# alexrich021/3dvnet

Measured on AMD Instinct MI355X. Metric: depth maps/sec (256x320, 96 planes, 7 src), higher is better.
Workload: dtype f32 storage/accumulate; MFMA operands split-bf16x3 (hi*hi+hi*lo+lo*hi, 16 mantissa bits); warp/variance f32 VALU; 1 GPU; cfg2: ScanNet-shape 256x320, 1 ref + 7 src (8 edges/ref), 96 planes, 56x56 plane grid, 32-ch quarter features 64x80; fused warp+variance -> CostRegNet -> soft-argmin depth (rows A1-A6); n_img_per_gpu=71, edges_per_ref=8, parallelism=single GPU, launch=eager, ranks_seen=1

## Files before the change

3dvnet_amd/build.py:

```python
import glob
import hashlib
import os
import subprocess
import sys

HERE = os.path.dirname(os.path.abspath(__file__))
ROOT = os.path.dirname(HERE)
CSRC = os.path.join(HERE, 'csrc')
LIB = os.path.join(HERE, 'lib3dvnet_hip.so')
HIPCC = os.environ.get('HIPCC', '/opt/rocm/bin/hipcc')
FLAGS = ['--offload-arch=gfx950', '-O3', '-std=c++17', '-fPIC', '-Wall', '-Wno-unused-function',
         '-I', os.path.join(ROOT, 'include'), '-I', CSRC] + os.environ.get('V3D_EXTRA_FLAGS', '').split()


def sources():
    return sorted(glob.glob(os.path.join(CSRC, '*.hip')))


def _flags_tag():
    return hashlib.sha256(' '.join([HIPCC] + FLAGS).encode()).hexdigest()[:12]


def _stale(target, deps):
    if not os.path.exists(target):
        return True
    t = os.path.getmtime(target)
    return any(os.path.getmtime(d) > t for d in deps)


def build(force=False, verbose=False, strict=False):
    headers = glob.glob(os.path.join(CSRC, '*.h')) + glob.glob(os.path.join(ROOT, 'include', '*.h'))
    tag = _flags_tag()
    objdir = os.path.join(HERE, 'build', tag)
    os.makedirs(objdir, exist_ok=True)
    stamp = os.path.join(HERE, 'build', 'linked_flags')
    linked = open(stamp).read().strip() if os.path.exists(stamp) else None
    procs, objs = [], []
    for src in sources():
        obj = os.path.join(objdir, os.path.basename(src)[:-4] + '.o')
        objs.append(obj)
        if force or _stale(obj, [src] + headers):
            cmd = [HIPCC] + FLAGS + ['-c', src, '-o', obj]
            if verbose:
                print(' '.join(cmd))
            procs.append((src, subprocess.Popen(cmd, stdout=subprocess.PIPE, stderr=subprocess.STDOUT)))
    for src, p in procs:
        out, _ = p.communicate()
        if p.returncode != 0:
            sys.stderr.write(out.decode())
            raise RuntimeError('hipcc failed on %s' % src)
        if verbose and out:
            print(out.decode())
    if not os.environ.get('V3D_EXTRA_FLAGS', '').strip() and not os.environ.get('V3D_SKIP_LDS_CHECK'):
        sys.path.insert(0, HERE)
        try:
            import isa_check
            isa_check.check(os.path.join(objdir, 'decoder.o'), strict=strict)
            isa_check.check_wide_lds(os.path.join(objdir, 'irb.o'), 'irb_kernel', strict=strict)
            isa_check.check_wide_lds(os.path.join(objdir, 'fpn.o'), 'fpn_level_kernel', strict=strict)
            isa_check.check_wide_lds(os.path.join(objdir, 'propz.o'), 'propz_kernel', strict=strict)
            isa_check.check_no_scratch(os.path.join(objdir, 'fusion.o'), 'fuse_depths_kernel', strict=strict)
            isa_check.check_no_scratch(os.path.join(objdir, 'tsdf.o'), 'tsdf_integrate_kernel', strict=strict)
            isa_check.check_no_scratch(os.path.join(objdir, 'tsdf_resample.o'), 'tsdf_resample_kernel', strict=strict)
            isa_check.check_no_scratch(os.path.join(objdir, 'tsdf_resample.o'), 'volume_resample_nearest_kernel', strict=strict)
            isa_check.check_no_scratch(os.path.join(objdir, 'cloudmetrics.o'), 'nn_query_kernel', strict=strict)
            isa_check.check_no_scratch(os.path.join(objdir, 'mesh.o'), 'mc_[a-z_]*_kernel', strict=strict)
            isa_check.check_no_scratch(os.path.join(objdir, 'meshrender.o'), 'mesh_render_kernel', strict=strict)
            isa_check.check_no_scratch(os.path.join(objdir, 'psv_variance.o'), 'psv_variance_window_kernel', strict=strict)
            isa_check.check_no_scratch(os.path.join(objdir, 'confidence.o'), 'soft_argmin_prob_kernel', strict=strict)
            isa_check.check_no_scratch(os.path.join(objdir, 'confidence.o'), 'prob_gather_kernel', strict=strict)
        finally:
            sys.path.pop(0)
    if force or procs or linked != tag or _stale(LIB, objs):
        cmd = [HIPCC, '--offload-arch=gfx950', '-shared', '-fPIC', '-o', LIB] + objs
        if verbose:
            print(' '.join(cmd))
        subprocess.check_call(cmd)
        with open(stamp, 'w') as f:
            f.write(tag + '\n')
    return LIB


if __name__ == '__main__':
    print(build(force='--force' in sys.argv, verbose='--verbose' in sys.argv))
```

3dvnet_amd/csrc/api.hip:

```cpp
#include <atomic>
#include <cstring>
#include <map>
#include <mutex>
#include <string>
#include <vector>

#include "v3d_common.h"

extern "C" int v3d_version(void) { return 9; }

extern "C" const char* v3d_last_error(void) { return v3d::err_buf(); }

namespace {
struct Span { std::string name; hipEvent_t a, b; };
std::mutex g_mu;
bool g_on = false;
std::vector<Span> g_spans;
std::vector<hipEvent_t> g_pool;
hipEvent_t take_event() {
  if (!g_pool.empty()) { hipEvent_t e = g_pool.back(); g_pool.pop_back(); return e; }
  hipEvent_t e; (void)hipEventCreate(&e); return e;
}
}

namespace v3d {
bool timing_enabled() { return g_on; }
void timing_begin(const char* name, hipStream_t s) {
  std::lock_guard<std::mutex> lk(g_mu);
  Span sp{name, take_event(), take_event()};
  (void)hipEventRecord(sp.a, s);
  g_spans.push_back(sp);
}
void timing_end(hipStream_t s) {
  std::lock_guard<std::mutex> lk(g_mu);
  if (!g_spans.empty()) (void)hipEventRecord(g_spans.back().b, s);
}
}

namespace {
struct OptDef { const char* name; int def; };
const OptDef kOptDefs[v3d::kOptCount] = {{"psv_kernel", 0}, {"c12_march", 1}, {"stop_after", 99}, {"gemm_rounds", 1},
                                         {"gemm_pipe", 1}, {"psv_walk", 0}, {"render_coop", 64}};
std::atomic<int> g_opt[v3d::kOptCount];
std::atomic<bool> g_opt_init{false};
void opt_init() {
  if (!g_opt_init.load(std::memory_order_acquire)) {
    std::lock_guard<std::mutex> lk(g_mu);
    if (!g_opt_init.load()) {
      for (int i = 0; i < v3d::kOptCount; ++i) g_opt[i].store(kOptDefs[i].def);
      g_opt_init.store(true, std::memory_order_release);
    }
  }
}
}

int v3d::option(v3d::Option o) {
  opt_init();
  return g_opt[o].load(std::memory_order_relaxed);
}

extern "C" int v3d_set_option(const char* name, int value) {
  V3D_REQUIRE(name, V3D_ERR_BAD_ARG, "v3d_set_option: null name");
  opt_init();
  for (int i = 0; i < v3d::kOptCount; ++i)
    if (!strcmp(name, kOptDefs[i].name)) {
      V3D_REQUIRE(!(i == v3d::kOptGemmRounds || i == v3d::kOptGemmPipe) || value == 0 || value == 1, V3D_ERR_BAD_ARG,
                  "v3d_set_option: %s must be 0 or 1 (got %d)", name, value);
      V3D_REQUIRE(!(i == v3d::kOptPsvWalk || i == v3d::kOptRenderCoop) || value >= 0, V3D_ERR_BAD_ARG,
                  "v3d_set_option: %s must be >= 0 (got %d)", name, value);
      g_opt[i].store(value);
      return V3D_OK;
    }
  return v3d::fail(V3D_ERR_BAD_ARG, "v3d_set_option: unknown option '%s'", name);
}

extern "C" int v3d_get_option(const char* name, int* value) {
  V3D_REQUIRE(name && value, V3D_ERR_BAD_ARG, "v3d_get_option: null argument");
  opt_init();
  for (int i = 0; i < v3d::kOptCount; ++i)
    if (!strcmp(name, kOptDefs[i].name)) { *value = g_opt[i].load(); return V3D_OK; }
  return v3d::fail(V3D_ERR_BAD_ARG, "v3d_get_option: unknown option '%s'", name);
}

extern "C" int v3d_timing_enable(int on) {
  std::lock_guard<std::mutex> lk(g_mu);
  g_on = on != 0;
  return V3D_OK;
}

extern "C" int v3d_timing_collect(int max_entries, char* names, int name_stride, float* total_ms,
                                  int* launches) {
  std::lock_guard<std::mutex> lk(g_mu);
  std::map<std::string, std::pair<float, int>> agg;
  std::vector<std::string> order;
  for (auto& sp : g_spans) {
    float ms = 0.f;
    if (hipEventSynchronize(sp.b) == hipSuccess) (void)hipEventElapsedTime(&ms, sp.a, sp.b);
    if (!agg.count(sp.name)) order.push_back(sp.name);
    agg[sp.name].first += ms;
    agg[sp.name].second += 1;
    g_pool.push_back(sp.a);
    g_pool.push_back(sp.b);
  }
  g_spans.clear();
  int n = 0;
  for (auto& k : order) {
    if (n >= max_entries) break;
    if (names && name_stride > 0) {
      strncpy(names + (size_t)n * name_stride, k.c_str(), name_stride - 1);
      names[(size_t)n * name_stride + name_stride - 1] = 0;
    }
    if (total_ms) total_ms[n] = agg[k].first;
    if (launches) launches[n] = agg[k].second;
    ++n;
  }
  return n;
}
```

3dvnet_amd/csrc/costreg.hip:

```cpp
#include <cstdlib>
#include <type_traits>
#include <vector>

#include "v3d_common.h"
#include "weight_pack.h"

#ifndef V3D_ABLATE
#define V3D_ABLATE 0
#endif

namespace {

typedef float f32x4 __attribute__((ext_vector_type(4)));
typedef float f32x2 __attribute__((ext_vector_type(2)));

enum { kConvS1 = 0, kConvS2 = 1, kDeconvS2 = 2, kConvS1Pair = 3 };

#ifdef V3D_PHASE_TIMING
constexpr int kPhaseSlots = 1 << 16;
__device__ unsigned long long g_phase[8 * kPhaseSlots];
#define PHASE_DECL                                  \
  long long ph_t = __builtin_readcyclecounter();    \
  long long ph_acc[8] = {0, 0, 0, 0, 0, 0, 0, 0}
#define PHASE_MARK(i)                                   \
// ... 754 lines not shown
        }
      }
      __syncthreads();
      const size_t out_plane = (size_t)p.Do * p.Ho * p.Wo;
      constexpr int QPR = C0::TW / 4, NQ = 8 * C0::TD * C0::TH * QPR;
#pragma unroll
      for (int k = 0; k < (NQ + NT - 1) / NT; ++k) {
        const int i = k * NT + tid;
        if (i >= NQ) break;
        const int co = i / (C0::TD * C0::TH * QPR), rem = i % (C0::TD * C0::TH * QPR);
        const int row = rem / QPR, q = rem % QPR;
        const int gz = oz0 + row / C0::TH, gy = oy0 + row % C0::TH, gx = ox0 + 4 * q;
        if (gz >= p.Do || gy >= p.Ho || gx >= p.Wo) continue;
        f32x4 v = *reinterpret_cast<const f32x4*>(os + co * OCS + row * C0::TW + 4 * q);
        const size_t o = ((size_t)n * 8 + co) * out_plane + ((size_t)gz * p.Ho + gy) * p.Wo + gx;
        if (gx + 3 < p.Wo && (p.Wo & 3) == 0) {
          if (p.skip) { const f32x4 sk = *reinterpret_cast<const f32x4*>(p.skip + o); v += sk; }
          *reinterpret_cast<f32x4*>(p.out + o) = v;
        } else {
          for (int e = 0; e < 4 && gx + e < p.Wo; ++e) p.out[o + e] = v[e] + (p.skip ? p.skip[o + e] : 0.f);
        }
      }
      PHASE_MARK(6);
    }
    cur = nxt;
  }
  PHASE_FLUSH;
}

enum { kOutF32 = 1, kOutSplit = 2 };

template <int CIN_, int COUT_, int STRIDE_, int WB_, int OUT_>
struct CG {
  static constexpr int CIN = CIN_, COUT = COUT_, S = STRIDE_, WB = WB_, OUT = OUT_;
  static constexpr int NCH = CIN / 8, NCG = COUT / 16;
  static constexpr int NRB = 16 / WB;
#ifndef V3D_CG_TD_S1
#define V3D_CG_TD_S1 4
#endif
#ifndef V3D_CG_TD_S2
#define V3D_CG_TD_S2 3
#endif
  static constexpr int TD = WB != 14 ? (S == 2 ? 2 : 4) : S == 2 ? V3D_CG_TD_S2 : V3D_CG_TD_S1, TH = 4 * NRB, TW = WB;
  static constexpr int NKZ = 3;
  static constexpr int ID = S * (TD - 1) + 3, IH = S * (TH - 1) + 3, IW = S * (TW - 1) + 3;
  static constexpr int NVOX = ID * IH * IW, NVOXP = NVOX + 8;
  static constexpr int WQ = NKZ * 3 * 2 * 64;
  static constexpr int NVO = TD * TH * TW;
  static constexpr int LPR = IW <= 16 ? 16 : 32, RPI = 256 / LPR;
  static constexpr int NROWS = 2 * ID * IH, NIT = (NROWS + RPI - 1) / RPI;
  static constexpr int NWIT = (WQ + 255) / 256;
  static constexpr size_t LDS_BYTES = (size_t)(2 * NVOXP + WQ) * 16;
  static constexpr bool PERSIST = NCH == 1;
  static constexpr int OCC = 2;
  static_assert(CIN % 8 == 0 && COUT % 16 == 0 && (WB == 14 || WB == 8), "shape");
  static_assert((size_t)NVO * 64 <= LDS_BYTES, "split output staging fits in the workgroup's LDS");
  static_assert((size_t)16 * (NVO + 2) * 4 <= LDS_BYTES, "fp32 output staging fits in the workgroup's LDS");
  static_assert((NROWS + RPI) * ID * IH < (1 << 20) && 4 * NVO * NVO < (1 << 20), "v3d::small_div ranges of the staging / output index");
};

struct ConvGParams {
  const void* in;
  const void* wp;
  const float* bias;
  float* out_f32;
  void* out_split;
  int n, Di, Hi, Wi, Do, Ho, Wo, ntz, nty, ntx;
  unsigned m_tx, m_ty, m_tz;
};

template <class C>
__global__ __launch_bounds__(256, C::OCC) void convg_bf16x2_kernel(ConvGParams p, const float* __restrict__ bias_r) {
  extern __shared__ __attribute__((aligned(16))) unsigned char smem[];
  u32x4* const xs = reinterpret_cast<u32x4*>(smem);
  u32x4* const wq = xs + 2 * C::NVOXP;
  const int tid = threadIdx.x, lane = tid & 63;
  const int wave = __builtin_amdgcn_readfirstlane(tid >> 6);
  const int kq = lane >> 4, jn = lane & 15;
  const size_t in_plane = (size_t)p.Di * p.Hi * p.Wi;
  const size_t out_plane = (size_t)p.Do * p.Ho * p.Wo;

  struct Item { int cg, n, oz0, oy0, ox0; };
  auto decode = [&](int t) __attribute__((always_inline)) {
    Item q;
    const unsigned t0 = (unsigned)t / C::NCG;
    q.cg = (int)((unsigned)t - t0 * C::NCG);
    const unsigned t1 = v3d::udiv_magic(t0, (unsigned)p.ntx, p.m_tx), t2 = v3d::udiv_magic(t1, (unsigned)p.nty, p.m_ty);
    const unsigned t3 = v3d::udiv_magic(t2, (unsigned)p.ntz, p.m_tz);
    q.ox0 = (int)(t0 - t1 * (unsigned)p.ntx) * C::TW;
    q.oy0 = (int)(t1 - t2 * (unsigned)p.nty) * C::TH;
    q.oz0 = (int)(t2 - t3 * (unsigned)p.ntz) * C::TD;
    q.n = (int)t3;
    return q;
  };
  const v3d::TileWalk walk = v3d::xcd_tile_walk(p.n * p.ntz * p.nty * p.ntx * C::NCG);
  if (walk.t >= walk.end) return;

  const int lrow = tid / C::LPR, lx = tid % C::LPR;
  const bool xok = lx < C::IW;
  u32x4 pre[C::NIT], wreg[C::NWIT];
  constexpr bool XPRE = C::PERSIST;
  auto issue = [&](const Item& q, int chunk) __attribute__((always_inline)) {
    const int iz0 = C::S * q.oz0 - 1, iy0 = C::S * q.oy0 - 1, sgx = C::S * q.ox0 - 1 + lx;
    const bool xin = xok && sgx >= 0 && sgx < p.Wi;
    const int sxc = min(max(sgx, 0), p.Wi - 1);
    const char* const ins = reinterpret_cast<const char*>(reinterpret_cast<const u32x4*>(p.in) +
                                                          ((size_t)q.n * C::NCH + chunk) * 2 * in_plane);
    const u32x4* const wg = reinterpret_cast<const u32x4*>(p.wp) + (size_t)q.cg * C::NCH * C::WQ;
#pragma unroll
    for (int it = 0; it < C::NIT; ++it) {
      const unsigned rr = (unsigned)(it * C::RPI + lrow);
      const unsigned part = v3d::small_div<C::ID * C::IH>(rr), rem = rr - part * (C::ID * C::IH);
      const unsigned rz = v3d::small_div<C::IH>(rem), ry = rem - rz * C::IH;
      const int gz = iz0 + (int)rz, gy = iy0 + (int)ry;
      const bool ok = rr < C::NROWS && xin && gz >= 0 && gz < p.Di && gy >= 0 && gy < p.Hi;
      const int zc = min(max(gz, 0), p.Di - 1), yc = min(max(gy, 0), p.Hi - 1);
      const unsigned idx = (part ? (unsigned)in_plane : 0u) + __umul24(__umul24(zc, p.Hi) + yc, p.Wi) + sxc;
      const u32x4 v = *reinterpret_cast<const u32x4*>(ins + idx * 16u);
      pre[it] = ok ? v : (u32x4){0u, 0u, 0u, 0u};
    }
#pragma unroll
    for (int i = 0; i < C::NWIT; ++i)
      wreg[i] = (i * 256 + tid < C::WQ) ? wg[(size_t)chunk * C::WQ + i * 256 + tid] : (u32x4){0u, 0u, 0u, 0u};
  };
  auto commit = [&]() __attribute__((always_inline)) {
#pragma unroll
    for (int it = 0; it < C::NIT; ++it) {
      const unsigned rr = (unsigned)(it * C::RPI + lrow);
      const unsigned part = v3d::small_div<C::ID * C::IH>(rr), rem = rr - part * (C::ID * C::IH);
      if (rr < C::NROWS && xok) xs[part * C::NVOXP + rem * C::IW + lx] = pre[it];
    }
#pragma unroll
    for (int i = 0; i < C::NWIT; ++i)
      if (i * 256 + tid < C::WQ) wq[i * 256 + tid] = wreg[i];
  };

  const int lr = jn / C::WB, lxo = jn % C::WB;
  f32x4 acc[C::TD];
  const u32x4* const wf = wq + lane;
  const int ly = wave * C::NRB + lr;
  const bool live = jn < C::NRB * C::WB;

  PHASE_DECL;
  Item cur = decode(walk.t);
  issue(cur, 0);
  PHASE_MARK(0);
#pragma unroll 1
  for (int t = walk.t; t < walk.end; t += walk.step) {
    const int tn = t + walk.step;
    const bool has_next = C::PERSIST && tn < walk.end;
    const Item nxt = decode(has_next ? tn : t);
#pragma unroll
    for (int z = 0; z < C::TD; ++z) acc[z] = (f32x4){0.f, 0.f, 0.f, 0.f};
#pragma unroll 1
    for (int chunk = 0; chunk < C::NCH; ++chunk) {
      __syncthreads();
      commit();
      if (chunk == 0 && tid < 16) xs[(tid >> 3) * C::NVOXP + C::NVOX + (tid & 7)] = (u32x4){0u, 0u, 0u, 0u};
      __syncthreads();
      PHASE_MARK(1);
      if (chunk + 1 < C::NCH) issue(cur, chunk + 1);
      else if (XPRE && has_next) issue(nxt, 0);
#ifndef V3D_CG_KYU
#define V3D_CG_KYU 1
#endif
#pragma unroll V3D_CG_KYU
      for (int ky = 0; ky < 3; ++ky) {
        bf16x8 a_hi[C::NKZ], a_lo[C::NKZ];
#pragma unroll
        for (int kz = 0; kz < C::NKZ; ++kz) {
          a_hi[kz] = __builtin_bit_cast(bf16x8, wf[((kz * 3 + ky) * 2) * 64]);
          a_lo[kz] = __builtin_bit_cast(bf16x8, wf[((kz * 3 + ky) * 2 + 1) * 64]);
        }
        const int rowbase = (C::S * (wave * C::NRB + lr) + ky) * C::IW + C::S * lxo + kq;
#pragma unroll
        for (int iz = 0; iz < C::ID; ++iz) {
          const bf16x8 b_hi = __builtin_bit_cast(bf16x8, xs[rowbase + iz * C::IH * C::IW]);
          const bf16x8 b_lo = __builtin_bit_cast(bf16x8, xs[rowbase + iz * C::IH * C::IW + C::NVOXP]);
#pragma unroll
          for (int kz = 0; kz < C::NKZ; ++kz) {
            const int z2 = iz - kz;
            if (z2 >= 0 && z2 % C::S == 0 && z2 / C::S < C::TD)
              acc[z2 / C::S] = __builtin_amdgcn_mfma_f32_16x16x32_bf16(a_hi[kz], b_hi, acc[z2 / C::S], 0, 0, 0);
          }
#pragma unroll
          for (int kz = 0; kz < C::NKZ; ++kz) {
            const int z2 = iz - kz;
            if (z2 >= 0 && z2 % C::S == 0 && z2 / C::S < C::TD)
              acc[z2 / C::S] = __builtin_amdgcn_mfma_f32_16x16x32_bf16(a_hi[kz], b_lo, acc[z2 / C::S], 0, 0, 0);
          }
#pragma unroll
          for (int kz = 0; kz < C::NKZ; ++kz) {
            const int z2 = iz - kz;
            if (z2 >= 0 && z2 % C::S == 0 && z2 / C::S < C::TD)
              acc[z2 / C::S] = __builtin_amdgcn_mfma_f32_16x16x32_bf16(a_lo[kz], b_hi, acc[z2 / C::S], 0, 0, 0);
          }
        }
      }
      PHASE_MARK(2);
    }
    __syncthreads();
    PHASE_MARK(3);

    const int cg = cur.cg, n = cur.n, oz0 = cur.oz0, oy0 = cur.oy0, ox0 = cur.ox0;
    float vout[C::TD][4];
    {
      float bias[4];
#pragma unroll
      for (int r = 0; r < 4; ++r) {
        const float b0 = bias_r[cg * 16 + r], b1 = bias_r[cg * 16 + 4 + r], b2 = bias_r[cg * 16 + 8 + r], b3 = bias_r[cg * 16 + 12 + r];
        bias[r] = lane_select(kq & 2, lane_select(kq & 1, b3, b2), lane_select(kq & 1, b1, b0));
      }
#pragma unroll
      for (int z = 0; z < C::TD; ++z)
#pragma unroll
        for (int r = 0; r < 4; ++r) vout[z][r] = fmaxf(acc[z][r] + bias[r], 0.f);
    }
    if constexpr ((C::OUT & kOutSplit) != 0) {
      u32x2* const sp2 = reinterpret_cast<u32x2*>(smem);
#pragma unroll
      for (int z = 0; z < C::TD; ++z) {
        if (!live) break;
        u32x2 hp, lp;
        split4(vout[z][0], vout[z][1], vout[z][2], vout[z][3], hp, lp);
        const int vox = (z * C::TH + ly) * C::TW + lxo;
        sp2[((((kq >> 1) * 2 + 0) * C::NVO) + vox) * 2 + (kq & 1)] = hp;
        sp2[((((kq >> 1) * 2 + 1) * C::NVO) + vox) * 2 + (kq & 1)] = lp;
      }
      __syncthreads();
      char* const outs = reinterpret_cast<char*>(reinterpret_cast<u32x4*>(p.out_split) + ((size_t)n * (C::COUT / 8) + cg * 2) * 2 * out_plane);
      const u32x4* const sq = reinterpret_cast<const u32x4*>(smem);
      for (int i = tid; i < 4 * C::NVO; i += 256) {
        const unsigned gp = v3d::small_div<C::NVO>((unsigned)i), vox = (unsigned)i - gp * C::NVO;
        const unsigned vz = v3d::small_div<C::TH * C::TW>(vox), vr = vox - vz * (C::TH * C::TW);
        const unsigned vy = v3d::small_div<C::TW>(vr), vx = vr - vy * C::TW;
        const int gz = oz0 + (int)vz, gy = oy0 + (int)vy, gx = ox0 + (int)vx;
        const unsigned idx = __umul24(gp, (unsigned)out_plane) + __umul24(__umul24(gz, p.Ho) + gy, p.Wo) + gx;
        if (gz < p.Do && gy < p.Ho && gx < p.Wo) *reinterpret_cast<u32x4*>(outs + idx * 16u) = sq[i];
      }
      if constexpr ((C::OUT & kOutF32) != 0) __syncthreads();
    }
    if constexpr ((C::OUT & kOutF32) != 0) {
      constexpr int OCS = C::NVO + 2;
      float* const os = reinterpret_cast<float*>(smem);
      if (live) {
#pragma unroll
        for (int z = 0; z < C::TD; ++z)
#pragma unroll
          for (int r = 0; r < 4; ++r) os[(4 * kq + r) * OCS + (z * C::TH + ly) * C::TW + lxo] = vout[z][r];
      }
      __syncthreads();
      constexpr int NR = C::TD * C::TH, QPR = C::TW / 2;
      for (int i = tid; i < 16 * NR * QPR; i += 256) {
        const int co = i / (NR * QPR), row = (i / QPR) % NR, q = i % QPR;
        const int gz = oz0 + row / C::TH, gy = oy0 + row % C::TH, gx = ox0 + 2 * q;
        if (gz >= p.Do || gy >= p.Ho || gx >= p.Wo) continue;
        const float2 v = *reinterpret_cast<const float2*>(os + co * OCS + row * C::TW + 2 * q);
        float* o = p.out_f32 + ((size_t)n * C::COUT + cg * 16 + co) * out_plane + ((size_t)gz * p.Ho + gy) * p.Wo + gx;
        if (gx + 1 < p.Wo && (p.Wo & 1) == 0) *reinterpret_cast<float2*>(o) = v;
        else { o[0] = v.x; if (gx + 1 < p.Wo) o[1] = v.y; }
      }
    }
    PHASE_MARK(4);
    if (!C::PERSIST) break;
    cur = nxt;
  }
  PHASE_FLUSH;
}

template <int CIN_, int COUT_, int WB_, int OUT_, bool SKIP_SPLIT_ = false>
struct DG {
  static constexpr int CIN = CIN_, COUT = COUT_, WB = WB_, OUT = OUT_;
  static constexpr bool SKIP_SPLIT = SKIP_SPLIT_;
  static constexpr int NCH = CIN / 8, NCG = COUT / 16;
  static constexpr int NRB = 16 / WB;
  static constexpr int CZ = 2, CY = 4 * NRB, CX = WB;
  static constexpr int VZ = CZ + 1, VY = CY + 1, VX = CX + 2;
  static constexpr int NVOX = VZ * VY * VX, NVOXP = NVOX + 8;
  static constexpr int WQ = 12 * 2 * 64;
  static constexpr int NSLOT = 2 * NVOX;
  static constexpr int NIT = (NSLOT + 255) / 256, NWIT = (WQ + 255) / 256;
  static constexpr int LDS_BYTES = (2 * NVOXP + WQ) * 16;
  static_assert(CIN % 8 == 0 && COUT % 16 == 0 && (WB == 14 || WB == 8), "shape");
  static_assert(LDS_BYTES <= 64 * 1024, "static LDS");
};

struct DeconvGParams {
  const void* in;
  const void* wp;
  const float* bias;
  const float* skip;
  float* out_f32;
  void* out_split;
  int n, Di, Hi, Wi, ntz, nty, ntx;
  unsigned m_tx, m_ty, m_tz;
};

template <class C>
__global__ __launch_bounds__(256, 2) void deconvg_bf16x2_kernel(DeconvGParams p) {
  __shared__ __attribute__((aligned(16))) unsigned char smem[C::LDS_BYTES];
  u32x4* const xs = reinterpret_cast<u32x4*>(smem);
  u32x4* const wq = xs + 2 * C::NVOXP;
  const int tid = threadIdx.x, lane = tid & 63;
  const int wave = __builtin_amdgcn_readfirstlane(tid >> 6);
  const int kq = lane >> 4, jn = lane & 15;
  const int cg = blockIdx.y;
  const unsigned b0 = (unsigned)v3d::xcd_contiguous_block();
  const unsigned b1 = v3d::udiv_magic(b0, (unsigned)p.ntx, p.m_tx), b2 = v3d::udiv_magic(b1, (unsigned)p.nty, p.m_ty);
  const unsigned b3 = v3d::udiv_magic(b2, (unsigned)p.ntz, p.m_tz);
  const int tx = (int)(b0 - b1 * (unsigned)p.ntx), ty = (int)(b1 - b2 * (unsigned)p.nty), tz = (int)(b2 - b3 * (unsigned)p.ntz);
  const int n = (int)b3;
  const int cz0 = tz * C::CZ, cy0 = ty * C::CY, cx0 = tx * C::CX;
  const int Do = 2 * p.Di, Ho = 2 * p.Hi, Wo = 2 * p.Wi;
  const size_t in_plane = (size_t)p.Di * p.Hi * p.Wi;
  const size_t out_plane = (size_t)Do * Ho * Wo;

  const u32x4* const ins = reinterpret_cast<const u32x4*>(p.in) + (size_t)n * C::NCH * 2 * in_plane;
  const u32x4* const wg = reinterpret_cast<const u32x4*>(p.wp) + (size_t)cg * C::NCH * C::WQ;
  u32x4 pre[C::NIT], wreg[C::NWIT];
  static_assert(C::NIT * 256 * C::NVOX < (1 << 20), "v3d::small_div range of the staging index");
// ... 577 lines not shown
#endif
constexpr int kC0Waves = V3D_C0_WAVES;
int launch_conv0_bf16(bool split_in, bool split_out, const float* in, const float* wbf, const float* bias, const float* skip, float* out, int n,
                      int Di, int Hi, int Wi, hipStream_t s) {
  ConvParams p;
  p.in = in; p.wp = wbf; p.bias = bias; p.skip = skip; p.out = out; p.n = n;
  p.Di = Di; p.Hi = Hi; p.Wi = Wi; p.Do = Di; p.Ho = Hi; p.Wo = Wi;
  p.ntz = (Di + C0::TD - 1) / C0::TD; p.nty = (Hi + C0::TH - 1) / C0::TH; p.ntx = (Wi + C0::TW - 1) / C0::TW;
  p.relu = 1;
  p.zy_order = tile_order(p.ntx, p.nty);
  const long long blocks = (long long)n * p.ntz * p.nty * p.ntx;
  V3D_REQUIRE(blocks > 0 && blocks < (1ll << 31), V3D_ERR_BAD_SHAPE, "conv0: bad grid");
  V3D_REQUIRE((long long)8 * Di * Hi * Wi < (1ll << 31), V3D_ERR_BAD_SHAPE, "conv0: input volume too large");
  static bool lds_opted[4][64] = {};
  const void* const kernels[4] = {(const void*)conv0_bf16x2_kernel<false, false, 4>, (const void*)conv0_bf16x2_kernel<true, false, 4>,
                                  (const void*)conv0_bf16x2_kernel<true, true, kC0Waves>, (const void*)conv0_bf16x2_kernel<false, true, 4>};
  for (int k = 0; k < 4; ++k)
    if (const int rc = v3d::opt_in_dynamic_lds(kernels[k], (int)C0::LDS_BYTES, lds_opted[k]); rc != V3D_OK) return rc;
  {
    v3d::TimedScope ts("costreg_conv0", s);
#ifdef V3D_C0_PERSIST
    const unsigned grid = v3d::persistent_grid(blocks, 2);
#else
    const unsigned grid = (unsigned)((blocks + 7) / 8 * 8);
#endif
    if (split_in && split_out) conv0_bf16x2_kernel<true, true, kC0Waves><<<grid, 64 * kC0Waves, C0::LDS_BYTES, s>>>(p);
    else if (split_in) conv0_bf16x2_kernel<true, false, 4><<<grid, 256, C0::LDS_BYTES, s>>>(p);
    else if (split_out) conv0_bf16x2_kernel<false, true, 4><<<grid, 256, C0::LDS_BYTES, s>>>(p);
    else conv0_bf16x2_kernel<false, false, 4><<<grid, 256, C0::LDS_BYTES, s>>>(p);
  }
  V3D_CHECK_LAUNCH("conv0_bf16x2_kernel");
  return V3D_OK;
}
}

namespace {
template <class C>
int launch_convg(const char* name, const void* in, const float* wbf, const float* bias, float* out_f32, void* out_split,
                 int n, int Di, int Hi, int Wi, hipStream_t s) {
  ConvGParams p;
  p.in = in; p.wp = wbf; p.bias = bias; p.out_f32 = out_f32; p.out_split = out_split; p.n = n;
  p.Di = Di; p.Hi = Hi; p.Wi = Wi;
  p.Do = (Di - 1) / C::S + 1; p.Ho = (Hi - 1) / C::S + 1; p.Wo = (Wi - 1) / C::S + 1;
  p.ntz = (p.Do + C::TD - 1) / C::TD; p.nty = (p.Ho + C::TH - 1) / C::TH; p.ntx = (p.Wo + C::TW - 1) / C::TW;
  const long long blocks = (long long)n * p.ntz * p.nty * p.ntx;
  V3D_REQUIRE(blocks > 0 && blocks < (1ll << 31), V3D_ERR_BAD_SHAPE, "%s: bad grid", name);
  V3D_REQUIRE(((C::OUT & kOutF32) == 0 || out_f32) && ((C::OUT & kOutSplit) == 0 || out_split), V3D_ERR_BAD_ARG,
              "%s: missing output buffer", name);
  p.m_tx = v3d::magic_u32((unsigned long long)blocks, (unsigned)p.ntx);
  p.m_ty = v3d::magic_u32((unsigned long long)blocks / p.ntx + 1, (unsigned)p.nty);
  p.m_tz = v3d::magic_u32((unsigned long long)blocks / p.ntx / p.nty + 1, (unsigned)p.ntz);
  V3D_REQUIRE(Di < (1 << 12) && Hi < (1 << 12) && Wi < (1 << 12) && (long long)Di * Hi * Wi < (1ll << 24), V3D_ERR_BAD_SHAPE,
              "%s: volume %d x %d x %d too large for 32-bit slot offsets", name, Di, Hi, Wi);
  static bool lds_opted[64] = {};
  if (const int rc = v3d::opt_in_dynamic_lds((const void*)convg_bf16x2_kernel<C>, (int)C::LDS_BYTES, lds_opted); rc != V3D_OK) return rc;
  {
    v3d::TimedScope ts(name, s);
    unsigned grid = (unsigned)((blocks * C::NCG + 7) / 8 * 8);
    if (C::PERSIST) {
      static int wgs_per_cu = 0;
      if (wgs_per_cu == 0) {
        int nb = 0;
        V3D_CHECK_HIP(hipOccupancyMaxActiveBlocksPerMultiprocessor(&nb, (const void*)convg_bf16x2_kernel<C>, 256, C::LDS_BYTES));
        wgs_per_cu = nb > 0 ? nb : 1;
      }
      grid = v3d::persistent_grid(blocks * C::NCG, wgs_per_cu);
    }
    convg_bf16x2_kernel<C><<<grid, 256, C::LDS_BYTES, s>>>(p, p.bias);
  }
  V3D_CHECK_LAUNCH(name);
  return V3D_OK;
}
}

namespace {
template <class C>
int launch_deconvg(const char* name, const void* in, const float* wbf, const float* bias, const float* skip, float* out_f32,
                   void* out_split, int n, int Di, int Hi, int Wi, hipStream_t s) {
  DeconvGParams p;
  p.in = in; p.wp = wbf; p.bias = bias; p.skip = skip; p.out_f32 = out_f32; p.out_split = out_split; p.n = n;
  p.Di = Di; p.Hi = Hi; p.Wi = Wi;
  p.ntz = (Di + C::CZ - 1) / C::CZ; p.nty = (Hi + C::CY - 1) / C::CY; p.ntx = (Wi + C::CX - 1) / C::CX;
  const long long blocks = (long long)n * p.ntz * p.nty * p.ntx;
  V3D_REQUIRE(blocks > 0 && blocks < (1ll << 31), V3D_ERR_BAD_SHAPE, "%s: bad grid", name);
  V3D_REQUIRE(skip && ((C::OUT & kOutF32) == 0 || out_f32) && ((C::OUT & kOutSplit) == 0 || out_split), V3D_ERR_BAD_ARG,
              "%s: missing buffer", name);
  V3D_REQUIRE(Di < (1 << 12) && Hi < (1 << 12) && Wi < (1 << 12) && (long long)Di * Hi * Wi < (1ll << 24), V3D_ERR_BAD_SHAPE,
              "%s: volume %d x %d x %d too large for 32-bit slot offsets", name, Di, Hi, Wi);
  p.m_tx = v3d::magic_u32((unsigned long long)blocks, (unsigned)p.ntx);
  p.m_ty = v3d::magic_u32((unsigned long long)blocks / p.ntx + 1, (unsigned)p.nty);
  p.m_tz = v3d::magic_u32((unsigned long long)blocks / p.ntx / p.nty + 1, (unsigned)p.ntz);
  {
    v3d::TimedScope ts(name, s);
    deconvg_bf16x2_kernel<C><<<dim3((unsigned)blocks, C::NCG), 256, 0, s>>>(p);
  }
  V3D_CHECK_LAUNCH(name);
  return V3D_OK;
}
}

struct v3d_costreg_weights {
  int in_channels, base;
  float* dev;
  size_t wp_ofs[10], bias_ofs[10], prob_w2_ofs, prob_b_ofs, c0bf_ofs, c0f32_ofs, cgbf_ofs[7], dgbf_ofs[2], c9bf_ofs, c9f32_ofs, total;
};

// ... 467 lines not shown
```

3dvnet_amd/csrc/v3d_common.h:

```cpp
#pragma once
#include <hip/hip_runtime.h>

#include <cstdarg>
#include <cstdio>
#include <cstring>

#include "v3d.h"

namespace v3d {

inline char* err_buf() {
  static thread_local char buf[512] = {0};
  return buf;
}

inline int fail(int code, const char* fmt, ...) {
  va_list ap;
  va_start(ap, fmt);
  vsnprintf(err_buf(), 512, fmt, ap);
  va_end(ap);
  return code;
}

#define V3D_CHECK_HIP(expr)                                                                    \
  do {                                                                                         \
    hipError_t e_ = (expr);                                                                    \
    if (e_ != hipSuccess)                                                                      \
      return v3d::fail(V3D_ERR_HIP, "%s failed: %s (%s:%d)", #expr, hipGetErrorString(e_),     \
                       __FILE__, __LINE__);                                                    \
  } while (0)

#define V3D_CHECK_LAUNCH(name)                                                                 \
  do {                                                                                         \
    hipError_t e_ = hipGetLastError();                                                         \
    if (e_ != hipSuccess)                                                                      \
      return v3d::fail(V3D_ERR_HIP, "launch of %s failed: %s", name, hipGetErrorString(e_));   \
  } while (0)

#define V3D_REQUIRE(cond, code, ...)                                                           \
  do {                                                                                         \
    if (!(cond)) return v3d::fail(code, __VA_ARGS__);                                          \
  } while (0)

inline size_t align_up(size_t x, size_t a) { return (x + a - 1) / a * a; }

enum Option {
  kOptPsvKernel,
  kOptC12March,
  kOptStopAfter,
  kOptGemmRounds,
  kOptGemmPipe,
  kOptPsvWalk,
  kOptRenderCoop,
  kOptCount
};
int option(Option o);

bool timing_enabled();
void timing_begin(const char* name, hipStream_t s);
void timing_end(hipStream_t s);

inline unsigned persistent_grid(long long n_tiles, int wgs_per_cu) {
  static int n_cu = 0;
  if (n_cu == 0) {
    int dev = 0, v = 0;
    if (hipGetDevice(&dev) != hipSuccess || hipDeviceGetAttribute(&v, hipDeviceAttributeMultiprocessorCount, dev) != hipSuccess || v <= 0) v = 256;
    n_cu = v;
  }
  long long g = (long long)n_cu * wgs_per_cu;
  if (g > n_tiles) g = n_tiles;
  g = (g + 7) / 8 * 8;
  return (unsigned)g;
}

inline int opt_in_dynamic_lds(const void* kernel, int bytes, bool* done_per_device) {
  int dev = 0;
  V3D_CHECK_HIP(hipGetDevice(&dev));
  V3D_REQUIRE(dev >= 0 && dev < 64, V3D_ERR_UNSUPPORTED, "device ordinal %d", dev);
  if (!done_per_device[dev]) {
    V3D_CHECK_HIP(hipFuncSetAttribute(kernel, hipFuncAttributeMaxDynamicSharedMemorySize, bytes));
    done_per_device[dev] = true;
  }
  return V3D_OK;
}

struct TimedScope {
  hipStream_t s;
  bool on;
  TimedScope(const char* name, hipStream_t s_) : s(s_), on(timing_enabled()) {
    if (on) timing_begin(name, s);
  }
  ~TimedScope() {
    if (on) timing_end(s);
  }
};

__device__ __forceinline__ int xcd_contiguous_block() {
  const int total = (int)gridDim.x, per = total >> 3, rem = total & 7;
  const int x = (int)blockIdx.x & 7, i = (int)blockIdx.x >> 3;
  return x * per + (x < rem ? x : rem) + i;
}

inline unsigned magic_u32(unsigned long long x_max, unsigned d) {
  if (d <= 1 || x_max * d >= (1ull << 32)) return 0u;
  return (unsigned)(((1ull << 32) + d - 1) / d);
}
// ... 92 lines not shown
```

Measured before the change: 19870 depth maps/s.

## Add direct global-to-LDS DMA variant of grouped 3D conv kernel

Result: no change. 20000 depth maps/s, median of 6 (+0.7%).

```diff
diff --git a/3dvnet_amd/build.py b/3dvnet_amd/build.py
--- a/3dvnet_amd/build.py
+++ b/3dvnet_amd/build.py
@@ -69,6 +69,7 @@
             isa_check.check_no_scratch(os.path.join(objdir, 'psv_variance.o'), 'psv_variance_window_kernel', strict=strict)
             isa_check.check_no_scratch(os.path.join(objdir, 'confidence.o'), 'soft_argmin_prob_kernel', strict=strict)
             isa_check.check_no_scratch(os.path.join(objdir, 'confidence.o'), 'prob_gather_kernel', strict=strict)
+            isa_check.check_no_scratch(os.path.join(objdir, 'costreg.o'), 'convg_(bf16x2|dma)_kernel', strict=strict)
         finally:
             sys.path.pop(0)
     if force or procs or linked != tag or _stale(LIB, objs):
diff --git a/3dvnet_amd/csrc/api.hip b/3dvnet_amd/csrc/api.hip
--- a/3dvnet_amd/csrc/api.hip
+++ b/3dvnet_amd/csrc/api.hip
@@ -40,7 +40,7 @@
 namespace {
 struct OptDef { const char* name; int def; };
 const OptDef kOptDefs[v3d::kOptCount] = {{"psv_kernel", 0}, {"c12_march", 1}, {"stop_after", 99}, {"gemm_rounds", 1},
-                                         {"gemm_pipe", 1}, {"psv_walk", 0}, {"render_coop", 64}};
+                                         {"gemm_pipe", 1}, {"psv_walk", 0}, {"render_coop", 64}, {"convg_staging", 2}};
 std::atomic<int> g_opt[v3d::kOptCount];
 std::atomic<bool> g_opt_init{false};
 void opt_init() {
@@ -68,6 +68,8 @@
                   "v3d_set_option: %s must be 0 or 1 (got %d)", name, value);
       V3D_REQUIRE(!(i == v3d::kOptPsvWalk || i == v3d::kOptRenderCoop) || value >= 0, V3D_ERR_BAD_ARG,
                   "v3d_set_option: %s must be >= 0 (got %d)", name, value);
+      V3D_REQUIRE(i != v3d::kOptConvgStaging || (value >= 0 && value <= 2), V3D_ERR_BAD_ARG,
+                  "v3d_set_option: %s must be 0, 1 or 2 (got %d)", name, value);
       g_opt[i].store(value);
       return V3D_OK;
     }
diff --git a/3dvnet_amd/csrc/costreg.hip b/3dvnet_amd/csrc/costreg.hip
--- a/3dvnet_amd/csrc/costreg.hip
+++ b/3dvnet_amd/csrc/costreg.hip
@@ -830,6 +830,8 @@
   static constexpr int NWIT = (WQ + 255) / 256;
   static constexpr size_t LDS_BYTES = (size_t)(2 * NVOXP + WQ) * 16;
   static constexpr bool PERSIST = NCH == 1;
+  static constexpr bool HAS_DMA = NCH >= 2 && NCG >= 2;
+  static constexpr bool DMA_SHIPS = HAS_DMA && COUT == 64;
   static constexpr int OCC = 2;
   static_assert(CIN % 8 == 0 && COUT % 16 == 0 && (WB == 14 || WB == 8), "shape");
   static_assert((size_t)NVO * 64 <= LDS_BYTES, "split output staging fits in the workgroup's LDS");
@@ -846,6 +848,125 @@
   int n, Di, Hi, Wi, Do, Ho, Wo, ntz, nty, ntx;
   unsigned m_tx, m_ty, m_tz;
 };
+
+struct CGItem { int cg, n, oz0, oy0, ox0; };
+template <class C>
+__device__ __forceinline__ CGItem cg_decode(const ConvGParams& p, int t) {
+  CGItem q;
+  const unsigned t0 = (unsigned)t / C::NCG;
+  q.cg = (int)((unsigned)t - t0 * C::NCG);
+  const unsigned t1 = v3d::udiv_magic(t0, (unsigned)p.ntx, p.m_tx), t2 = v3d::udiv_magic(t1, (unsigned)p.nty, p.m_ty);
+  const unsigned t3 = v3d::udiv_magic(t2, (unsigned)p.ntz, p.m_tz);
+  q.ox0 = (int)(t0 - t1 * (unsigned)p.ntx) * C::TW;
+  q.oy0 = (int)(t1 - t2 * (unsigned)p.nty) * C::TH;
+  q.oz0 = (int)(t2 - t3 * (unsigned)p.ntz) * C::TD;
+  q.n = (int)t3;
+  return q;
+}
+
+template <class C>
+__device__ __forceinline__ void cg_mfma_chunk(const u32x4* xs, const u32x4* wf, int row0, f32x4 (&acc)[C::TD]) {
+#ifndef V3D_CG_KYU
+#define V3D_CG_KYU 1
+#endif
+#pragma unroll V3D_CG_KYU
+  for (int ky = 0; ky < 3; ++ky) {
+    bf16x8 a_hi[C::NKZ], a_lo[C::NKZ];
+#pragma unroll
+    for (int kz = 0; kz < C::NKZ; ++kz) {
+      a_hi[kz] = __builtin_bit_cast(bf16x8, wf[((kz * 3 + ky) * 2) * 64]);
+      a_lo[kz] = __builtin_bit_cast(bf16x8, wf[((kz * 3 + ky) * 2 + 1) * 64]);
+    }
+    const int rowbase = row0 + ky * C::IW;
+#pragma unroll
+    for (int iz = 0; iz < C::ID; ++iz) {
+      const bf16x8 b_hi = __builtin_bit_cast(bf16x8, xs[rowbase + iz * C::IH * C::IW]);
+      const bf16x8 b_lo = __builtin_bit_cast(bf16x8, xs[rowbase + iz * C::IH * C::IW + C::NVOXP]);
+#pragma unroll
+      for (int kz = 0; kz < C::NKZ; ++kz) {
+        const int z2 = iz - kz;
+        if (z2 >= 0 && z2 % C::S == 0 && z2 / C::S < C::TD)
+          acc[z2 / C::S] = __builtin_amdgcn_mfma_f32_16x16x32_bf16(a_hi[kz], b_hi, acc[z2 / C::S], 0, 0, 0);
+      }
+#pragma unroll
+      for (int kz = 0; kz < C::NKZ; ++kz) {
+        const int z2 = iz - kz;
+        if (z2 >= 0 && z2 % C::S == 0 && z2 / C::S < C::TD)
+          acc[z2 / C::S] = __builtin_amdgcn_mfma_f32_16x16x32_bf16(a_hi[kz], b_lo, acc[z2 / C::S], 0, 0, 0);
+      }
+#pragma unroll
+      for (int kz = 0; kz < C::NKZ; ++kz) {
+        const int z2 = iz - kz;
+        if (z2 >= 0 && z2 % C::S == 0 && z2 / C::S < C::TD)
+          acc[z2 / C::S] = __builtin_amdgcn_mfma_f32_16x16x32_bf16(a_lo[kz], b_hi, acc[z2 / C::S], 0, 0, 0);
+      }
+    }
+  }
+}
+
+template <class C>
+__device__ __forceinline__ void cg_epilogue(const ConvGParams& p, const float* __restrict__ bias_r, unsigned char* stage, int cg,
+                                            int n, int oz0, int oy0, int ox0, const f32x4 (&acc)[C::TD], int tid, int kq, int ly,
+                                            int lxo, bool live, size_t out_plane) {
+  float vout[C::TD][4];
+  {
+    float bias[4];
+#pragma unroll
+    for (int r = 0; r < 4; ++r) {
+      const float b0 = bias_r[cg * 16 + r], b1 = bias_r[cg * 16 + 4 + r], b2 = bias_r[cg * 16 + 8 + r], b3 = bias_r[cg * 16 + 12 + r];
+      bias[r] = lane_select(kq & 2, lane_select(kq & 1, b3, b2), lane_select(kq & 1, b1, b0));
+    }
+#pragma unroll
+    for (int z = 0; z < C::TD; ++z)
+#pragma unroll
+      for (int r = 0; r < 4; ++r) vout[z][r] = fmaxf(acc[z][r] + bias[r], 0.f);
+  }
+  if constexpr ((C::OUT & kOutSplit) != 0) {
+    u32x2* const sp2 = reinterpret_cast<u32x2*>(stage);
+#pragma unroll
+    for (int z = 0; z < C::TD; ++z) {
+      if (!live) break;
+      u32x2 hp, lp;
+      split4(vout[z][0], vout[z][1], vout[z][2], vout[z][3], hp, lp);
+      const int vox = (z * C::TH + ly) * C::TW + lxo;
+      sp2[((((kq >> 1) * 2 + 0) * C::NVO) + vox) * 2 + (kq & 1)] = hp;
+      sp2[((((kq >> 1) * 2 + 1) * C::NVO) + vox) * 2 + (kq & 1)] = lp;
+    }
+    __syncthreads();
+    char* const outs = reinterpret_cast<char*>(reinterpret_cast<u32x4*>(p.out_split) + ((size_t)n * (C::COUT / 8) + cg * 2) * 2 * out_plane);
+    const u32x4* const sq = reinterpret_cast<const u32x4*>(stage);
+    for (int i = tid; i < 4 * C::NVO; i += 256) {
+      const unsigned gp = v3d::small_div<C::NVO>((unsigned)i), vox = (unsigned)i - gp * C::NVO;
+      const unsigned vz = v3d::small_div<C::TH * C::TW>(vox), vr = vox - vz * (C::TH * C::TW);
+      const unsigned vy = v3d::small_div<C::TW>(vr), vx = vr - vy * C::TW;
+      const int gz = oz0 + (int)vz, gy = oy0 + (int)vy, gx = ox0 + (int)vx;
+      const unsigned idx = __umul24(gp, (unsigned)out_plane) + __umul24(__umul24(gz, p.Ho) + gy, p.Wo) + gx;
+      if (gz < p.Do && gy < p.Ho && gx < p.Wo) *reinterpret_cast<u32x4*>(outs + idx * 16u) = sq[i];
+    }
+    if constexpr ((C::OUT & kOutF32) != 0) __syncthreads();
+  }
+  if constexpr ((C::OUT & kOutF32) != 0) {
+    constexpr int OCS = C::NVO + 2;
+    float* const os = reinterpret_cast<float*>(stage);
+    if (live) {
+#pragma unroll
+      for (int z = 0; z < C::TD; ++z)
+#pragma unroll
+        for (int r = 0; r < 4; ++r) os[(4 * kq + r) * OCS + (z * C::TH + ly) * C::TW + lxo] = vout[z][r];
+    }
+    __syncthreads();
+    constexpr int NR = C::TD * C::TH, QPR = C::TW / 2;
+    for (int i = tid; i < 16 * NR * QPR; i += 256) {
+      const int co = i / (NR * QPR), row = (i / QPR) % NR, q = i % QPR;
+      const int gz = oz0 + row / C::TH, gy = oy0 + row % C::TH, gx = ox0 + 2 * q;
+      if (gz >= p.Do || gy >= p.Ho || gx >= p.Wo) continue;
+      const float2 v = *reinterpret_cast<const float2*>(os + co * OCS + row * C::TW + 2 * q);
+      float* o = p.out_f32 + ((size_t)n * C::COUT + cg * 16 + co) * out_plane + ((size_t)gz * p.Ho + gy) * p.Wo + gx;
+      if (gx + 1 < p.Wo && (p.Wo & 1) == 0) *reinterpret_cast<float2*>(o) = v;
+      else { o[0] = v.x; if (gx + 1 < p.Wo) o[1] = v.y; }
+    }
+  }
+}
 
 template <class C>
 __global__ __launch_bounds__(256, C::OCC) void convg_bf16x2_kernel(ConvGParams p, const float* __restrict__ bias_r) {
@@ -858,19 +979,8 @@
   const size_t in_plane = (size_t)p.Di * p.Hi * p.Wi;
   const size_t out_plane = (size_t)p.Do * p.Ho * p.Wo;
 
-  struct Item { int cg, n, oz0, oy0, ox0; };
-  auto decode = [&](int t) __attribute__((always_inline)) {
-    Item q;
-    const unsigned t0 = (unsigned)t / C::NCG;
-    q.cg = (int)((unsigned)t - t0 * C::NCG);
-    const unsigned t1 = v3d::udiv_magic(t0, (unsigned)p.ntx, p.m_tx), t2 = v3d::udiv_magic(t1, (unsigned)p.nty, p.m_ty);
-    const unsigned t3 = v3d::udiv_magic(t2, (unsigned)p.ntz, p.m_tz);
-    q.ox0 = (int)(t0 - t1 * (unsigned)p.ntx) * C::TW;
-    q.oy0 = (int)(t1 - t2 * (unsigned)p.nty) * C::TH;
-    q.oz0 = (int)(t2 - t3 * (unsigned)p.ntz) * C::TD;
-    q.n = (int)t3;
-    return q;
-  };
+  using Item = CGItem;
+  auto decode = [&](int t) __attribute__((always_inline)) { return cg_decode<C>(p, t); };
   const v3d::TileWalk walk = v3d::xcd_tile_walk(p.n * p.ntz * p.nty * p.ntx * C::NCG);
   if (walk.t >= walk.end) return;
 
@@ -939,111 +1049,164 @@
       PHASE_MARK(1);
       if (chunk + 1 < C::NCH) issue(cur, chunk + 1);
       else if (XPRE && has_next) issue(nxt, 0);
-#ifndef V3D_CG_KYU
-#define V3D_CG_KYU 1
-#endif
-#pragma unroll V3D_CG_KYU
-      for (int ky = 0; ky < 3; ++ky) {
-        bf16x8 a_hi[C::NKZ], a_lo[C::NKZ];
-#pragma unroll
-        for (int kz = 0; kz < C::NKZ; ++kz) {
-          a_hi[kz] = __builtin_bit_cast(bf16x8, wf[((kz * 3 + ky) * 2) * 64]);
-          a_lo[kz] = __builtin_bit_cast(bf16x8, wf[((kz * 3 + ky) * 2 + 1) * 64]);
-        }
-        const int rowbase = (C::S * (wave * C::NRB + lr) + ky) * C::IW + C::S * lxo + kq;
-#pragma unroll
-        for (int iz = 0; iz < C::ID; ++iz) {
-          const bf16x8 b_hi = __builtin_bit_cast(bf16x8, xs[rowbase + iz * C::IH * C::IW]);
-          const bf16x8 b_lo = __builtin_bit_cast(bf16x8, xs[rowbase + iz * C::IH * C::IW + C::NVOXP]);
-#pragma unroll
-          for (int kz = 0; kz < C::NKZ; ++kz) {
-            const int z2 = iz - kz;
-            if (z2 >= 0 && z2 % C::S == 0 && z2 / C::S < C::TD)
-              acc[z2 / C::S] = __builtin_amdgcn_mfma_f32_16x16x32_bf16(a_hi[kz], b_hi, acc[z2 / C::S], 0, 0, 0);
-          }
-#pragma unroll
-          for (int kz = 0; kz < C::NKZ; ++kz) {
-            const int z2 = iz - kz;
-            if (z2 >= 0 && z2 % C::S == 0 && z2 / C::S < C::TD)
-              acc[z2 / C::S] = __builtin_amdgcn_mfma_f32_16x16x32_bf16(a_hi[kz], b_lo, acc[z2 / C::S], 0, 0, 0);
-          }
-#pragma unroll
-          for (int kz = 0; kz < C::NKZ; ++kz) {
-            const int z2 = iz - kz;
-            if (z2 >= 0 && z2 % C::S == 0 && z2 / C::S < C::TD)
-              acc[z2 / C::S] = __builtin_amdgcn_mfma_f32_16x16x32_bf16(a_lo[kz], b_hi, acc[z2 / C::S], 0, 0, 0);
-          }
-        }
-      }
+      cg_mfma_chunk<C>(xs, wf, C::S * ly * C::IW + C::S * lxo + kq, acc);
       PHASE_MARK(2);
     }
     __syncthreads();
     PHASE_MARK(3);
 
-    const int cg = cur.cg, n = cur.n, oz0 = cur.oz0, oy0 = cur.oy0, ox0 = cur.ox0;
-    float vout[C::TD][4];
-    {
-      float bias[4];
-#pragma unroll
-      for (int r = 0; r < 4; ++r) {
-        const float b0 = bias_r[cg * 16 + r], b1 = bias_r[cg * 16 + 4 + r], b2 = bias_r[cg * 16 + 8 + r], b3 = bias_r[cg * 16 + 12 + r];
-        bias[r] = lane_select(kq & 2, lane_select(kq & 1, b3, b2), lane_select(kq & 1, b1, b0));
-      }
-#pragma unroll
-      for (int z = 0; z < C::TD; ++z)
-#pragma unroll
-        for (int r = 0; r < 4; ++r) vout[z][r] = fmaxf(acc[z][r] + bias[r], 0.f);
-    }
-    if constexpr ((C::OUT & kOutSplit) != 0) {
-      u32x2* const sp2 = reinterpret_cast<u32x2*>(smem);
-#pragma unroll
-      for (int z = 0; z < C::TD; ++z) {
-        if (!live) break;
-        u32x2 hp, lp;
-        split4(vout[z][0], vout[z][1], vout[z][2], vout[z][3], hp, lp);
-        const int vox = (z * C::TH + ly) * C::TW + lxo;
-        sp2[((((kq >> 1) * 2 + 0) * C::NVO) + vox) * 2 + (kq & 1)] = hp;
-        sp2[((((kq >> 1) * 2 + 1) * C::NVO) + vox) * 2 + (kq & 1)] = lp;
-      }
-      __syncthreads();
-      char* const outs = reinterpret_cast<char*>(reinterpret_cast<u32x4*>(p.out_split) + ((size_t)n * (C::COUT / 8) + cg * 2) * 2 * out_plane);
-      const u32x4* const sq = reinterpret_cast<const u32x4*>(smem);
-      for (int i = tid; i < 4 * C::NVO; i += 256) {
-        const unsigned gp = v3d::small_div<C::NVO>((unsigned)i), vox = (unsigned)i - gp * C::NVO;
-        const unsigned vz = v3d::small_div<C::TH * C::TW>(vox), vr = vox - vz * (C::TH * C::TW);
-        const unsigned vy = v3d::small_div<C::TW>(vr), vx = vr - vy * C::TW;
-        const int gz = oz0 + (int)vz, gy = oy0 + (int)vy, gx = ox0 + (int)vx;
-        const unsigned idx = __umul24(gp, (unsigned)out_plane) + __umul24(__umul24(gz, p.Ho) + gy, p.Wo) + gx;
-        if (gz < p.Do && gy < p.Ho && gx < p.Wo) *reinterpret_cast<u32x4*>(outs + idx * 16u) = sq[i];
-      }
-      if constexpr ((C::OUT & kOutF32) != 0) __syncthreads();
-    }
-    if constexpr ((C::OUT & kOutF32) != 0) {
-      constexpr int OCS = C::NVO + 2;
-      float* const os = reinterpret_cast<float*>(smem);
-      if (live) {
-#pragma unroll
-        for (int z = 0; z < C::TD; ++z)
-#pragma unroll
-          for (int r = 0; r < 4; ++r) os[(4 * kq + r) * OCS + (z * C::TH + ly) * C::TW + lxo] = vout[z][r];
-      }
-      __syncthreads();
-      constexpr int NR = C::TD * C::TH, QPR = C::TW / 2;
-      for (int i = tid; i < 16 * NR * QPR; i += 256) {
-        const int co = i / (NR * QPR), row = (i / QPR) % NR, q = i % QPR;
-        const int gz = oz0 + row / C::TH, gy = oy0 + row % C::TH, gx = ox0 + 2 * q;
-        if (gz >= p.Do || gy >= p.Ho || gx >= p.Wo) continue;
-        const float2 v = *reinterpret_cast<const float2*>(os + co * OCS + row * C::TW + 2 * q);
-        float* o = p.out_f32 + ((size_t)n * C::COUT + cg * 16 + co) * out_plane + ((size_t)gz * p.Ho + gy) * p.Wo + gx;
-        if (gx + 1 < p.Wo && (p.Wo & 1) == 0) *reinterpret_cast<float2*>(o) = v;
-        else { o[0] = v.x; if (gx + 1 < p.Wo) o[1] = v.y; }
-      }
-    }
+    cg_epilogue<C>(p, bias_r, smem, cur.cg, cur.n, cur.oz0, cur.oy0, cur.ox0, acc, tid, kq, ly, lxo, live, out_plane);
     PHASE_MARK(4);
     if (!C::PERSIST) break;
     cur = nxt;
   }
   PHASE_FLUSH;
+}
+
+template <class C>
+struct CGD {
+  static constexpr int NRUN = (C::NVOX + 63) / 64, K = (NRUN + 3) / 4;
+  static constexpr int NWRUN = C::WQ / 64, KW = (NWRUN + 3) / 4;
+  static constexpr int BUF_BYTES = (2 * C::NVOXP + C::WQ) * 16;
+  static constexpr size_t LDS_BYTES = BUF_BYTES;
+  static constexpr int STAGE_OFS = 2 * C::NVOXP * 16;
+  static constexpr int STAGE_BYTES = BUF_BYTES - STAGE_OFS;
+  static_assert(C::WQ % 64 == 0, "shape");
+  static_assert(4 * K * 64 * C::IW < (1 << 20) && (4 * K * 64 / C::IW + 1) * C::IH < (1 << 20), "v3d::small_div ranges of the slot index");
+  static_assert(C::NVO * 64 <= STAGE_BYTES && 16 * (C::NVO + 2) * 4 <= STAGE_BYTES, "output staging fits");
+  static_assert(LDS_BYTES <= 80 * 1024, "two workgroups per CU");
+};
+
+template <class C>
+__global__ __launch_bounds__(256, C::OCC) void convg_dma_kernel(ConvGParams p, const float* __restrict__ bias_r) {
+  using G = CGD<C>;
+  extern __shared__ __attribute__((aligned(16))) unsigned char smem[];
+  const unsigned smem_lds = __builtin_amdgcn_readfirstlane((unsigned)(size_t)(__attribute__((address_space(3))) void*)smem);
+  const int tid = threadIdx.x, lane = tid & 63;
+  const int wave = __builtin_amdgcn_readfirstlane(tid >> 6);
+  const int kq = lane >> 4, jn = lane & 15;
+  const size_t in_plane = (size_t)p.Di * p.Hi * p.Wi;
+  const size_t out_plane = (size_t)p.Do * p.Ho * p.Wo;
+
+  const v3d::TileWalk walk = v3d::xcd_tile_walk(p.n * p.ntz * p.nty * p.ntx * C::NCG);
+  if (walk.t >= walk.end) return;
+
+  unsigned voff[G::K];
+  unsigned long long vmask[G::K];
+  const unsigned lane16 = (unsigned)lane * 16u;
+  auto setup = [&](const CGItem& q) __attribute__((always_inline)) {
+    const int iz0 = C::S * q.oz0 - 1, iy0 = C::S * q.oy0 - 1, ix0 = C::S * q.ox0 - 1;
+#pragma unroll
+    for (int k = 0; k < G::K; ++k) {
+      const unsigned sl = (unsigned)(wave + 4 * k) * 64u + (unsigned)lane;
+      const unsigned row = v3d::small_div<C::IW>(sl), lx = sl - row * C::IW;
+      const unsigned rz = v3d::small_div<C::IH>(row), ry = row - rz * C::IH;
+      const int gz = iz0 + (int)rz, gy = iy0 + (int)ry, gx = ix0 + (int)lx;
+      const bool ok = sl < (unsigned)C::NVOX && gz >= 0 && gz < p.Di && gy >= 0 && gy < p.Hi && gx >= 0 && gx < p.Wi;
+      voff[k] = ok ? (__umul24(__umul24(gz, p.Hi) + gy, p.Wi) + (unsigned)gx) * 16u : 0u;
+      vmask[k] = __ballot(ok);
+    }
+  };
+  auto zero_fill = [&]() __attribute__((always_inline)) {
+    u32x4* const xb = reinterpret_cast<u32x4*>(smem);
+#pragma unroll
+    for (int k = 0; k < G::K; ++k) {
+      const unsigned sl = (unsigned)(wave + 4 * k) * 64u + (unsigned)lane;
+      if (sl < (unsigned)C::NVOX && ((vmask[k] >> lane) & 1ull) == 0) {
+        xb[sl] = (u32x4){0u, 0u, 0u, 0u};
+        xb[C::NVOXP + sl] = (u32x4){0u, 0u, 0u, 0u};
+      }
+    }
+    if (tid < 16) xb[(tid >> 3) * C::NVOXP + C::NVOX + (tid & 7)] = (u32x4){0u, 0u, 0u, 0u};
+  };
+  auto issue_x = [&](const CGItem& q, int chunk) __attribute__((always_inline)) {
+    const char* const bh = reinterpret_cast<const char*>(reinterpret_cast<const u32x4*>(p.in) +
+                                                         ((size_t)q.n * C::NCH + chunk) * 2 * in_plane);
+    const char* const bl = bh + in_plane * 16;
+    const unsigned dst = smem_lds + (unsigned)wave * 1024u;
+#pragma unroll
+    for (int k = 0; k < G::K; ++k) {
+      if (vmask[k] == 0) continue;
+      unsigned long long sv;
+      unsigned m0v;
+      asm volatile(
+          "s_mov_b64 %[sv], exec\n\t"
+          "s_mov_b32 %[m0v], m0\n\t"
+          "s_mov_b32 m0, %[dh]\n\t"
+          "s_mov_b64 exec, %[k]\n\t"
+          "global_load_lds_dwordx4 %[v], %[bh]\n\t"
+          "s_mov_b32 m0, %[dl]\n\t"
+          "s_nop 0\n\t"
+          "global_load_lds_dwordx4 %[v], %[bl]\n\t"
+          "s_mov_b64 exec, %[sv]\n\t"
+          "s_mov_b32 m0, %[m0v]"
+          : [sv] "=&s"(sv), [m0v] "=&s"(m0v)
+          : [dh] "s"(dst + (unsigned)k * 4096u), [dl] "s"(dst + (unsigned)k * 4096u + (unsigned)C::NVOXP * 16u), [bh] "s"(bh),
+            [bl] "s"(bl), [v] "v"(voff[k]), [k] "s"(vmask[k])
+          : "memory", "scc");
+    }
+  };
+  auto issue_w = [&](const CGItem& q, int chunk) __attribute__((always_inline)) {
+    const char* const wg = reinterpret_cast<const char*>(reinterpret_cast<const u32x4*>(p.wp) +
+                                                         ((size_t)q.cg * C::NCH + chunk) * C::WQ);
+    const unsigned dst = smem_lds + 2u * C::NVOXP * 16u;
+#pragma unroll
+    for (int k = 0; k < G::KW; ++k) {
+      const int r = wave + 4 * k;
+      if (r >= G::NWRUN) continue;
+      unsigned keep;
+      asm volatile("s_mov_b32 %0, m0\n\ts_mov_b32 m0, %3\n\ts_nop 0\n\tglobal_load_lds_dwordx4 %1, %2\n\ts_mov_b32 m0, %0"
+                   : "=&s"(keep) : "v"(lane16), "s"(wg + r * 1024), "s"(dst + (unsigned)r * 1024u) : "memory");
+    }
+  };
+  auto landed_barrier = [&]() __attribute__((always_inline)) {
+    asm volatile("s_waitcnt vmcnt(0)" ::: "memory");
+    __syncthreads();
+  };
+
+  const int lr = jn / C::WB, lxo = jn % C::WB;
+  f32x4 acc[C::TD];
+  const int ly = wave * C::NRB + lr;
+  const bool live = jn < C::NRB * C::WB;
+  const int row0 = C::S * ly * C::IW + C::S * lxo + kq;
+
+  CGItem cur = cg_decode<C>(p, walk.t);
+  setup(cur);
+  zero_fill();
+  issue_x(cur, 0);
+  issue_w(cur, 0);
+  landed_barrier();
+#pragma unroll 1
+  for (int t = walk.t; t < walk.end; t += walk.step) {
+    const int tn = t + walk.step;
+    const bool has_next = tn < walk.end;
+    const CGItem nxt = cg_decode<C>(p, has_next ? tn : t);
+#pragma unroll
+    for (int z = 0; z < C::TD; ++z) acc[z] = (f32x4){0.f, 0.f, 0.f, 0.f};
+#pragma unroll 1
+    for (int chunk = 0; chunk < C::NCH; ++chunk) {
+      const u32x4* const xs = reinterpret_cast<const u32x4*>(smem);
+      cg_mfma_chunk<C>(xs, xs + 2 * C::NVOXP + lane, row0, acc);
+      __syncthreads();
+      if (chunk + 1 < C::NCH) {
+        issue_x(cur, chunk + 1);
+        issue_w(cur, chunk + 1);
+        landed_barrier();
+      } else if (has_next) {
+        setup(nxt);
+        zero_fill();
+        issue_x(nxt, 0);
+      }
+    }
+    cg_epilogue<C>(p, bias_r, smem + G::STAGE_OFS, cur.cg, cur.n, cur.oz0, cur.oy0, cur.ox0, acc, tid, kq, ly,
+                   lxo, live, out_plane);
+    if (!has_next) break;
+    __syncthreads();
+    issue_w(nxt, 0);
+    landed_barrier();
+    cur = nxt;
+  }
+  asm volatile("s_waitcnt vmcnt(0)" ::: "memory");
 }
 
 template <int CIN_, int COUT_, int WB_, int OUT_, bool SKIP_SPLIT_ = false>
@@ -1727,6 +1890,24 @@
   p.m_tz = v3d::magic_u32((unsigned long long)blocks / p.ntx / p.nty + 1, (unsigned)p.ntz);
   V3D_REQUIRE(Di < (1 << 12) && Hi < (1 << 12) && Wi < (1 << 12) && (long long)Di * Hi * Wi < (1ll << 24), V3D_ERR_BAD_SHAPE,
               "%s: volume %d x %d x %d too large for 32-bit slot offsets", name, Di, Hi, Wi);
+  if constexpr (C::HAS_DMA) {
+    const int staging = v3d::option(v3d::kOptConvgStaging);
+    if (staging == 1 || (staging != 0 && C::DMA_SHIPS)) {
+      using G = CGD<C>;
+      static bool dma_opted[64] = {};
+      if (const int rc = v3d::opt_in_dynamic_lds((const void*)convg_dma_kernel<C>, (int)G::LDS_BYTES, dma_opted); rc != V3D_OK) return rc;
+      v3d::TimedScope ts(name, s);
+      static int wgs_per_cu = 0;
+      if (wgs_per_cu == 0) {
+        int nb = 0;
+        V3D_CHECK_HIP(hipOccupancyMaxActiveBlocksPerMultiprocessor(&nb, (const void*)convg_dma_kernel<C>, 256, G::LDS_BYTES));
+        wgs_per_cu = nb > 0 ? nb : 1;
+      }
+      convg_dma_kernel<C><<<v3d::persistent_grid(blocks * C::NCG, wgs_per_cu), 256, G::LDS_BYTES, s>>>(p, p.bias);
+      V3D_CHECK_LAUNCH(name);
+      return V3D_OK;
+    }
+  }
   static bool lds_opted[64] = {};
   if (const int rc = v3d::opt_in_dynamic_lds((const void*)convg_bf16x2_kernel<C>, (int)C::LDS_BYTES, lds_opted); rc != V3D_OK) return rc;
   {
diff --git a/3dvnet_amd/csrc/v3d_common.h b/3dvnet_amd/csrc/v3d_common.h
--- a/3dvnet_amd/csrc/v3d_common.h
+++ b/3dvnet_amd/csrc/v3d_common.h
@@ -52,6 +52,7 @@
   kOptGemmPipe,
   kOptPsvWalk,
   kOptRenderCoop,
+  kOptConvgStaging,
   kOptCount
 };
 int option(Option o);
```
